# fegennari/3DWorld

Measured on AMD Instinct MI355X. Metric: heightmap Gcells/sec (noise+erosion), 16384^2 grid, higher is better.
Workload: dtype f32

## Files before the change

### 3dworld_amd/csrc/terra_common.hpp

```cpp
#pragma once
#include <stdint.h>
#include <math.h>
#include <float.h>
#include <limits.h>
#include <string.h>

#if defined(__HIPCC__)
#include <hip/hip_runtime.h>
#define TERRA_HD __host__ __device__ __forceinline__
#define TERRA_D  __device__ __forceinline__
#define TERRA_HD_COLD __host__ __device__ __attribute__((noinline))
#define TERRA_LAMBDA __host__ __device__
#else
#define TERRA_HD inline
#define TERRA_HD_COLD inline
#define TERRA_D  inline
#define TERRA_LAMBDA
#endif

#define TERRA_LIKELY(x)   __builtin_expect(!!(x), 1)
#define TERRA_UNLIKELY(x) __builtin_expect(!!(x), 0)

namespace terra {

constexpr int   F_TABLE_SIZE   = 90;
constexpr int   NUM_FREQ_COMP  = 9;
constexpr int   N_RAND_SIN2    = 10;
constexpr int   TSIZE          = 1 << 15;
constexpr float PI_F           = 3.141592654f;
constexpr int   EROSION_PAD    = 4;

TERRA_HD constexpr int sg_chunk_len(int kstart, int KC) {int const nk = F_TABLE_SIZE - kstart, n = (nk + KC - 1)/KC; return (nk > 0 && n > 0) ? (nk + n - 1)/n : 0;}
TERRA_HD constexpr int sg_chunk_last_row(int k0, int kn) {return k0 + kn - 1 + (kn & 1);}
TERRA_HD constexpr int sg_last_row_read(int kstart, int KC) {
	int const per = sg_chunk_len(kstart, KC);
	int last = -1;
	for (int k0 = kstart; per > 0 && k0 < F_TABLE_SIZE; k0 += per) {
		int const kn = (k0 + per > F_TABLE_SIZE) ? F_TABLE_SIZE - k0 : per, l = sg_chunk_last_row(k0, kn);
		if (l > last) {last = l;}
	}
	return last;
}
constexpr int SG_TABLE_ROWS = F_TABLE_SIZE + 1;
constexpr bool sg_table_rows_suffice() {
	constexpr int kcs[3] = {20, 27, 45};
	for (int i = 0; i < 3; ++i) {for (int kstart = 0; kstart <= F_TABLE_SIZE; ++kstart) {if (sg_last_row_read(kstart, kcs[i]) >= SG_TABLE_ROWS) return false;}}
	return true;
}
static_assert(sg_table_rows_suffice(), "k_sine_grid's staging would read behind the sine tables");

enum {MGEN_SINE = 0, MGEN_SIMPLEX, MGEN_PERLIN, MGEN_SIMPLEX_GPU, MGEN_DWARP_GPU};

TERRA_HD float min_std(float a, float b) {return (b < a) ? b : a;}
TERRA_HD float max_std(float a, float b) {return (a < b) ? b : a;}
TERRA_HD uint32_t f2ord(float f) {uint32_t u; memcpy(&u, &f, 4); return (u & 0x80000000u) ? ~u : (u | 0x80000000u);}
TERRA_HD float ord2f(uint32_t o) {uint32_t u = (o & 0x80000000u) ? (o & 0x7FFFFFFFu) : ~o; float f; memcpy(&f, &u, 4); return f;}
TERRA_HD int   imin(int a, int b) {return (b < a) ? b : a;}
TERRA_HD int   imax(int a, int b) {return (a < b) ? b : a;}
TERRA_HD float clip01(float x)  {return max_std(0.0f, min_std(1.0f, x));}
TERRA_HD float clip_pm1(float x) {return max_std(-1.0f, min_std(1.0f, x));}
TERRA_HD int f2i_x86(float f) {return (f >= -2147483648.0f && f < 2147483648.0f) ? (int)f : INT_MIN;}
TERRA_HD int d2i_x86(double v) {return (v > -2147483649.0 && v < 2147483648.0) ? (int)v : INT_MIN;}
TERRA_HD uint32_t f2u_x86(float f) {return (f > -9223372036854775808.0f && f < 9223372036854775808.0f) ? (uint32_t)(uint64_t)(int64_t)f : 0u;}
TERRA_HD uint32_t d2u_x86(double d) {return (d > -9223372036854775808.0 && d < 9223372036854775808.0) ? (uint32_t)(uint64_t)(int64_t)d : 0u;}
TERRA_HD int add_wrap(int a, int b) {return (int)((uint32_t)a + (uint32_t)b);}
TERRA_HD int sub_wrap(int a, int b) {return (int)((uint32_t)a - (uint32_t)b);}
TERRA_HD int abs_x86(int v) {return (v < 0) ? (int)(0u - (uint32_t)v) : v;}

struct shadow_pt_t {float x, y, z;};
TERRA_HD int shadow_region(shadow_pt_t v, float const d[3][2]) {
	int region = 0;
	if (v.x < d[0][0]) {region |= 0x01;} else if (v.x >= d[0][1]) {region |= 0x02;}
	if (v.y < d[1][0]) {region |= 0x04;} else if (v.y >= d[1][1]) {region |= 0x08;}
	if (v.z < d[2][0]) {region |= 0x10;} else if (v.z >= d[2][1]) {region |= 0x20;}
	return region;
}
TERRA_HD bool shadow_line_clip(shadow_pt_t &v1, shadow_pt_t &v2, float const d[3][2]) {
	int const region1 = shadow_region(v1, d), region2 = shadow_region(v2, d);
	if (region1 & region2) return false;
	int const region3 = region1 | region2;
	if (region3 == 0) return true;
	float tmin = 0.0f, tmax = 1.0f;
	shadow_pt_t const dv = {v2.x - v1.x, v2.y - v1.y, v2.z - v1.z};
#define TERRA_SH_CLIP(reg, va, vb, vd, vc) if (region3 & (reg)) {float const t = ((va) - (vb))/(vd); if ((vc) > 0.0f) {if (t > tmin) tmin = t;} else {if (t < tmax) tmax = t;} if (tmin >= tmax) return false;}
	TERRA_SH_CLIP(0x01, d[0][0], v1.x, dv.x,  dv.x)
	TERRA_SH_CLIP(0x02, d[0][1], v1.x, dv.x, -dv.x)
	TERRA_SH_CLIP(0x04, d[1][0], v1.y, dv.y,  dv.y)
	TERRA_SH_CLIP(0x08, d[1][1], v1.y, dv.y, -dv.y)
	TERRA_SH_CLIP(0x10, d[2][0], v1.z, dv.z,  dv.z)
	TERRA_SH_CLIP(0x20, d[2][1], v1.z, dv.z, -dv.z)
#undef TERRA_SH_CLIP
	if ((double)tmax > 1.0E-12) {v2.x = v1.x + dv.x*tmax; v2.y = v1.y + dv.y*tmax; v2.z = v1.z + dv.z*tmax;}
	if ((double)tmin < (1.0 - 1.0E-12)) {v1.x += dv.x*tmin; v1.y += dv.y*tmin; v1.z += dv.z*tmin;}
	return true;
}
template<class REMOVED, class MOVE> TERRA_HD uint32_t remove_elements_serial(uint32_t size, REMOVED removed, MOVE move) {
	for (uint32_t i = 0; i < size; ++i) {
		if (!removed(i)) continue;
		move(i, size - 1);
		--size;
		--i;
	}
	return size;
}

struct rand_gen_t {
	int64_t rseed1, rseed2;
	TERRA_HD void set_state(int64_t s1, int64_t s2) {rseed1 = s1; rseed2 = s2;}
	TERRA_HD void advance() {
		if ((rseed1 = 40014*(rseed1%53668) - 12211*(rseed1/53668)) < 0) rseed1 += 2147483563;
		if ((rseed2 = 40692*(rseed2%52774) - 3791 *(rseed2/52774)) < 0) rseed2 += 2147483399;
	}
	TERRA_HD int rand() {
		advance();
		int v = (int)rseed1 - (int)rseed2;
		if (v < 1) v += 2147483562;
		return v;
	}
	TERRA_HD double randd() {
		advance();
		double v = (double)rseed1 - (double)rseed2;
		if (v < 1) v += 2147483562;
		return v/2147483563.;
	}
	TERRA_HD float rand_float() {return (float)(0.000001*(rand()%1000000));}
	TERRA_HD float rand_uniform(float a, float b) {return a + (b - a)*(float)randd();}
};

struct sin_lut_t {
	float const *tab;
	float sscale;
	TERRA_HD int st_scale(float v) const {return f2i_x86(sscale*v) & (TSIZE-1);}
// ... 19 lines not shown
```

### 3dworld_amd/csrc/terra_hip.hip

```cpp
#include "terra_kernels.hpp"
#include "terra_fused.hpp"
#include "terra_fz_api.hpp"
#include "terra_simple_paths.hpp"
#include "terra_xfer.hpp"
#include <stdlib.h>

#define TERRA_HIP_CHECK(expr) do {hipError_t const e_ = (expr); if (e_ != hipSuccess) {throw std::runtime_error(std::string(#expr) + ": " + hipGetErrorString(e_));}} while (0)

struct hip_backend_t : terra::simple_paths<hip_backend_t> {
	int device = -1;
	hipStream_t stream = nullptr, own_stream = nullptr;
	hipEvent_t ev0 = nullptr, ev1 = nullptr;
	static constexpr bool has_kernels = true;
	terra::options_t const *opt = nullptr;
	int num_cus = 256;
	terra::dev_buf_t tile_pad, tile_order, tile_acc, tile_map, vox_p, h3_tab;
	template<class F> void for_each_buf(F f) {for (terra::dev_buf_t *b : {&tile_pad, &tile_order, &tile_acc, &tile_map, &vox_p, &h3_tab}) {f(*b);}}

	static int device_count() {int n = 0; if (hipGetDeviceCount(&n) != hipSuccess) return 0; return n;}
	void init(int dev) {
		device = dev;
		TERRA_HIP_CHECK(hipSetDevice(dev));
		TERRA_HIP_CHECK(hipStreamCreateWithFlags(&own_stream, hipStreamNonBlocking));
		stream = own_stream;
// ... 166 lines not shown
	template<class F> static void with_noise_mode(int md, F f) {
		switch (md) {
		case terra::MGEN_PERLIN:      f(std::integral_constant<int, terra::MGEN_PERLIN>()); break;
		case terra::MGEN_DWARP_GPU:   f(std::integral_constant<int, terra::MGEN_DWARP_GPU>()); break;
		case terra::MGEN_SIMPLEX_GPU: f(std::integral_constant<int, terra::MGEN_SIMPLEX_GPU>()); break;
		default:                      f(std::integral_constant<int, terra::MGEN_SIMPLEX>()); break;
		}
	}

	template<class F> void launch(size_t n, F f, int block = 256) {
		if (n == 0) return;
		use();
		size_t const nblocks = (n + block - 1)/block;
		if (nblocks > 0x7FFFFFFFull) throw std::invalid_argument("launch: grid too large");
		run(terra::k_generic<F>, dim3((unsigned)nblocks), dim3(block), 0, n, f);
	}

	template<class F> void launch_waves(size_t n, F f) {
		if (n == 0) return;
		use();
		if (n > 0x7FFFFFFFull) throw std::invalid_argument("launch_waves: grid too large");
		run(terra::k_waves<F>, dim3((unsigned)n), dim3(64), 0, f, 0u);
	}

	template<class F> void launch_waves_lean(size_t n, F f) {
		if (n == 0) return;
		use();
		if (n > 0x7FFFFFFFull) throw std::invalid_argument("launch_waves: grid too large");
		run(terra::k_waves_lean<F>, dim3((unsigned)n), dim3(64), 0, f);
	}

	template<class F> void launch_waves_nolds(size_t n, F f) {
		if (n == 0) return;
		use();
		if (n > 0x7FFFFFFFull) throw std::invalid_argument("launch_waves: grid too large");
		run(terra::k_waves_nolds<F>, dim3((unsigned)n), dim3(64), 0, f);
	}

	static float h3_scale(float amax) {int e = 0; if (amax > 0.0f && amax < 3.0e38f) {(void)frexpf(amax, &e);} return ldexpf(1.0f, 14 - e);}
	template<int KIND> bool sine_grid_h3(terra::sgf_job_t J, float amax_x, float amax_y, float const *vox_tab = nullptr, uint32_t vnx = 0, uint32_t vny = 0) {
		int const nk = (J.kstart < J.kend) ? J.kend - J.kstart : 0;
		uint32_t const nchunks = (uint32_t)((3*nk + 15)/16);
		if ((uint64_t)std::max(J.nxp, J.nyp)*32u*(nchunks + 1) >= 0xFFFFFFFFull) return false;
		size_t const bx = (size_t)nchunks*J.nxp*32u, by = (size_t)nchunks*J.nyp*32u;
		float const sx = h3_scale(amax_x), sy = h3_scale(amax_y);
		J.xh = h3_tab.grow(*this, bx + by + 64); J.yh = (char const *)J.xh + bx; J.nchunks = nchunks; J.unscale = 1.0f/(sx*sy);
		if (nchunks && vox_tab) {
			run(terra::k_split_voxel_table<false, terra::VOX_SINES>, dim3((J.nxp + 255)/256), dim3(256), 0, vox_tab, vnx, vny, J.nx, J.nxp, sx, (terra::sgh_u4 *)J.xh);
			run(terra::k_split_voxel_table<true, terra::VOX_SINES>, dim3((J.nyp + 255)/256), dim3(256), 0, vox_tab, vnx, vny, J.nx, J.nyp, sy, (terra::sgh_u4 *)J.yh);
		}
		else if (nchunks) {
			run(terra::k_split_table<false>, dim3((unsigned)(((size_t)nchunks*J.nxp + 255)/256)), dim3(256), 0, J.xt, J.nxp, J.kstart, J.kend, nchunks, sx, (terra::sgh_u4 *)J.xh);
			run(terra::k_split_table<true>, dim3((unsigned)(((size_t)nchunks*J.nyp + 255)/256)), dim3(256), 0, J.yt, J.nyp, J.kstart, J.kend, nchunks, sy, (terra::sgh_u4 *)J.yh);
		}
		if (KIND == terra::SGF_VOXELS && J.nx <= 64 && (J.nyp % 256u) == 0) {J.narrow = 1; J.ntx = 1; J.nty = J.nyp/256u;}
		unsigned const nb = J.ntx*J.nty, grid = ((nb + 7)/8)*8;
		run(terra::k_sine_grid_h3<KIND>, dim3(grid), dim3(256), 0, J);
		return true;
	}
	terra::sgf_job_t make_sgf_job(terra::grid_job_t const &job, terra::noise_consts_t const &nc, float const *xt, float const *yt, float const *smx, float const *smy, float *out, uint32_t *mm, unsigned ntx, unsigned nty) const {
		terra::sgf_job_t J; memset(&J, 0, sizeof(J));
		J.xt = xt; J.yt = yt; J.smx = smx; J.smy = smy; J.out = out; J.mm = mm; J.nx = job.nx; J.ny = job.ny; J.nxp = job.nxp; J.nyp = job.nyp; J.ntx = ntx; J.nty = nty; J.rowgroup = (unsigned)opt->sg_rowgroup;
		J.kstart = job.kstart; J.kend = terra::F_TABLE_SIZE; J.glaciate = (job.glaciate && nc.glaciate) ? 1 : 0; J.sine_mag = (job.glaciate && job.use_sine_mag) ? 1 : 0;
		J.zmax_est = nc.zmax_est; J.zmax_est2 = nc.zmax_est2; J.zmax_est2_inv = nc.zmax_est2_inv; J.sine_offset = job.sine_offset;
		return J;
	}
	bool sine_grid(terra::grid_job_t const &job, terra::noise_consts_t const &nc, terra::sin_lut_t const &L, float const *xt, float const *yt, float const *smx, float const *smy, float *out, uint32_t *mm) {
		if (opt->simple_kernels) {sine_grid_simple(job, nc, L, xt, yt, smx, smy, out); return false;}
		use();
		unsigned const ntx = job.nxp/terra::SG_BX, nty_all = (job.ny + terra::SG_BY - 1)/terra::SG_BY;
		if ((job.tyn || job.ty0) && (job.fused || job.tyn == 0 || job.ty0 >= nty_all || job.tyn > nty_all - job.ty0)) throw std::invalid_argument("sine_grid: a tile-row window must lie inside the grid (the fused kernels take whole grids only)");
		unsigned const nty = job.tyn ? job.tyn : nty_all;
		unsigned const nb = ntx*nty, grid = ((nb + 7)/8)*8;
		if (job.fused) {
			terra::sgf_job_t const J = make_sgf_job(job, nc, xt, yt, smx, smy, out, mm, ntx, nty);
			if (job.fused == 2 && sine_grid_h3<terra::SGF_GRID>(J, 1.0f, job.fast_amax)) return true;
			run(terra::k_sine_grid_mx<terra::SGF_GRID>, dim3(std::min(grid, (unsigned)(2*num_cus + 7)/8*8)), dim3(256), 0, J);
			return true;
		}
		terra::sg_tiles_t const tl{nullptr, nullptr, 0, (unsigned)opt->sg_rowgroup, 0, 0, 0, 0xFFFFFFFFu, 0, 0xFFFFFFFFu, 0};
		if (job.plain_only) {
			auto const go = [&](auto kern) {run(kern, dim3(grid), dim3(terra::SG_THREADS), 0, job, nc, L, xt, yt, smx, smy, out, ntx, nty, mm, tl);};
			if ((job.nx & 3u) == 0) {
				if (opt->sg_kc == 27) go(terra::k_sine_grid<false, false, 27>); else if (opt->sg_kc == 20) go(terra::k_sine_grid<false, false, 20>); else go(terra::k_sine_grid<false, false, 45>);
			}
			else {
				if (opt->sg_kc == 27) go(terra::k_sine_grid<false, false, 27, false>); else if (opt->sg_kc == 20) go(terra::k_sine_grid<false, false, 20, false>); else go(terra::k_sine_grid<false, false, 45, false>);
			}
		}
		else                {run(terra::k_sine_grid<false, true>, dim3(grid), dim3(terra::SG_THREADS), 0, job, nc, L, xt, yt, smx, smy, out, ntx, nty, mm, tl);}
		return true;
	}
	bool noise_grid(terra::grid_job_t const &job, terra::noise_consts_t const &nc, terra::sin_lut_t const &L, float const *smx, float const *smy, float *out, uint32_t *mm, uint32_t const *nlut) {
		if (opt->simple_kernels) {noise_grid_simple(job, nc, L, smx, smy, out); return false;}
		use();
		if (job.fused) {TERRA_HIP_CHECK((hipError_t)terra_fz_noise_grid(job.mode, &job, &nc, &L, smx, smy, out, mm, nlut, (void *)stream)); return true;}
		dim3 const grid((job.nx + 127)/128, (job.ny + terra::NG_ROWS - 1)/terra::NG_ROWS), block(256);
		terra::noise_oct_t const oc = terra::make_noise_oct(nc);
		with_noise_mode(job.mode, [&](auto m) {run(terra::k_noise_grid<decltype(m)::value>, grid, block, 0, job, nc, L, smx, smy, out, mm, nlut, oc);});
		return true;
	}
	bool tile_band_ok(uint32_t n, uint32_t nux, uint32_t nuy, uint32_t twx, bool unique_tiles, bool plain_only, int md) const {
		return !opt->simple_kernels && md == terra::MGEN_SINE && unique_tiles && plain_only && (uint64_t)n*2 >= (uint64_t)nux*nuy && ((nux*twx) & 3u) == 0 && opt->sg_kc_tiles == 27 && opt->ao_bands != 0;
	}
	void tile_grid(uint32_t n, terra::tile_ref_pod_t const *refs, uint32_t nux, uint32_t nuy, float const *xt, float const *yt, uint32_t nxpv, uint32_t nypv, float const *d_sm, float const *d_m0,
		int md, int shp, int kstart, bool use_sm, float so, terra::noise_consts_t const &nc, terra::sin_lut_t const &L, float dxv, float dyv, float *zvals, bool plain_only, uint32_t tw, bool unique_tiles, bool glaciate = true, uint32_t const *nlut = nullptr, int fused = 0, float fast_amax = 0.0f,
		terra::tile_band_t const *band = nullptr)
	{
		if (!opt->simple_kernels && md != terra::MGEN_SINE) {
			use();
			terra::grid_job_t job;
			job.mx0 = 0; job.my0 = 0; job.mdx = dxv; job.mdy = dyv; job.nx = job.ny = tw; job.nxp = nxpv; job.nyp = nypv;
			job.mode = md; job.shape = shp; job.kstart = kstart; job.glaciate = glaciate ? 1 : 0; job.use_sine_mag = use_sm ? 1 : 0; job.sine_offset = so; job.plain_only = 0;
			if (fused) {TERRA_HIP_CHECK((hipError_t)terra_fz_noise_tiles(refs, n, nux, d_sm, d_m0, &job, &nc, &L, zvals, tw, nlut, (void *)stream)); return;}
			terra::noise_oct_t const oc = terra::make_noise_oct(nc);
			size_t const threads = (size_t)n*tw*((tw + 1)/2);
			dim3 const grid((unsigned)((threads + 255)/256)), block(256);
			with_noise_mode(md, [&](auto m) {run(terra::k_noise_tiles<decltype(m)::value>, grid, block, 0, refs, n, nux, d_sm, d_m0, job, nc, L, zvals, tw, nlut, oc);});
			return;
		}
		if (opt->simple_kernels || md != terra::MGEN_SINE || !unique_tiles || (uint64_t)n*2 < (uint64_t)nux*nuy || ((uintptr_t)zvals & 7)) {tile_grid_simple(n, refs, nux, nuy, xt, yt, nxpv, nypv, d_sm, d_m0, md, shp, kstart, use_sm, so, nc, L, dxv, dyv, zvals, tw, glaciate, fused); return;}
		use();
		size_t const cnt = (size_t)nux*nuy;
		int32_t *tm = (int32_t *)tile_map.grow(*this, cnt*sizeof(int32_t));
		fill32(tm, 0xFFFFFFFFu, cnt);
		launch(n, [=] TERRA_LAMBDA (size_t i) {terra::tile_ref_pod_t const r = refs[i]; tm[(size_t)r.yi*nux + r.xi] = (int32_t)i;});
		terra::grid_job_t job;
		job.mx0 = 0; job.my0 = 0; job.mdx = dxv; job.mdy = dyv; job.nx = nux*tw; job.ny = nuy*(band ? band->twy : tw); job.nxp = nxpv; job.nyp = nypv;
		job.mode = terra::MGEN_SINE; job.shape = shp; job.kstart = kstart; job.glaciate = glaciate ? 1 : 0; job.use_sine_mag = use_sm ? 1 : 0; job.sine_offset = so;
		unsigned const ntx = job.nxp/terra::SG_BX, nty = (job.ny + terra::SG_BY - 1)/terra::SG_BY, nb = ntx*nty, grid = ((nb + 7)/8)*8;
		terra::sg_tiles_t tl{tm, d_m0, nux, (unsigned)opt->sg_rowgroup, tw, tw, tw, 0xFFFFFFFFu, 0, 0xFFFFFFFFu, 0};
		if (band) {tl.twy = band->twy; tl.ostride = band->ostride; tl.xsplit = band->xsplit; tl.xgap = band->xgap; tl.ysplit = band->ysplit; tl.ygap = band->ygap; fused = 0;}
		job.plain_only = plain_only ? 1 : 0;
		if (fused && plain_only) {
			terra::sgf_job_t J = make_sgf_job(job, nc, xt, yt, d_sm, d_sm + (size_t)nux*tw, zvals, nullptr, ntx, nty);
			J.tile_map = tm; J.nux = nux; J.tw = tw;
			if (fused == 2 && sine_grid_h3<terra::SGF_TILES>(J, 1.0f, fast_amax)) return;
			run(terra::k_sine_grid_mx<terra::SGF_TILES>, dim3(std::min(grid, (unsigned)(2*num_cus + 7)/8*8)), dim3(256), 0, J);
			return;
		}
		int const kc_tiles = opt->sg_kc_tiles;
		if (plain_only && kc_tiles == 27) {run(terra::k_sine_grid<true, false, 27>, dim3(grid), dim3(terra::SG_THREADS), 0, job, nc, L, xt, yt, d_sm, d_sm + (size_t)nux*tw, zvals, ntx, nty, (uint32_t *)nullptr, tl);}
		else if (plain_only) {run(terra::k_sine_grid<true, false>, dim3(grid), dim3(terra::SG_THREADS), 0, job, nc, L, xt, yt, d_sm, d_sm + (size_t)nux*tw, zvals, ntx, nty, (uint32_t *)nullptr, tl);}
		else            {run(terra::k_sine_grid<true, true>, dim3(grid), dim3(terra::SG_THREADS), 0, job, nc, L, xt, yt, d_sm, d_sm + (size_t)nux*tw, zvals, ntx, nty, (uint32_t *)nullptr, tl);}
	}
	terra::shadow_consts_t lanes_key; uint32_t lanes_np = 0; bool lanes_ok = false; terra::shadow_lanes_t lanes_cached;
	bool shadow_lanes(terra::shadow_consts_t const &c, uint32_t np, terra::shadow_lanes_t &lanes) {
		if (lanes_np != np || memcmp(&lanes_key, &c, sizeof(c)) != 0) {
			memset(&lanes_key, 0, sizeof(lanes_key)); memcpy(&lanes_key, &c, sizeof(c)); lanes_np = np;
			lanes_ok = terra::shadow_lane_order(c, np, terra::SH_LEVEL_THREADS, lanes_cached.path);
		}
		lanes = lanes_cached;
		return lanes_ok;
	}
	bool shadow_kernels_ok(terra::shadow_consts_t const &c, uint8_t const *sm, uint32_t np, terra::shadow_lanes_t &lanes) {
		return !opt->simple_kernels && c.xsize == 130 && !((uintptr_t)sm & 3) && shadow_lanes(c, np, lanes);
	}
	bool tile_shadows_flow(terra::shadow_consts_t const &c, uint32_t ntiles, uint32_t nslots, uint32_t const *ord, int32_t const *adj, float const *z, unsigned long long *out, uint8_t *sm, uint32_t np, uint32_t *sync_words) {
		terra::shadow_lanes_t lanes;
		if (opt->shadows_levels || !shadow_kernels_ok(c, sm, np, lanes)) return false;
		use();
		fill32(sync_words, 0u, 1);
		unsigned const grid = std::min<unsigned>(ntiles, (unsigned)(2*num_cus));
		run(terra::k_tile_shadows_flow, dim3(grid), dim3(terra::SH_LEVEL_THREADS), terra::SH_LEVEL_LDS, c, nslots, ntiles, ord, adj, z, out, sm, np, sync_words, lanes);
		return true;
	}
	void tile_shadows(terra::shadow_consts_t const &c, uint32_t cnt, uint32_t const *ord, int32_t const *adj, uint32_t n, float const *z, unsigned long long *out, uint8_t *sm, uint32_t np) {
// ... 354 lines not shown
```

### 3dworld_amd/csrc/terra_kernels.hpp

```cpp
#pragma once
#include "terra_driver.hpp"
#include "terra_noise_kernels.hpp"

namespace terra {

typedef float    st_f4 __attribute__((ext_vector_type(4)));
typedef uint32_t st_u4 __attribute__((ext_vector_type(4)));

template<class F> __global__ void k_generic(size_t n, F f) {
	size_t const i = (size_t)blockIdx.x*blockDim.x + threadIdx.x;
	if (i < n) {f(i);}
}

template<class F> __global__ __launch_bounds__(64) void k_waves(F f, unsigned first) {
	__builtin_amdgcn_s_setprio(3);
	__shared__ __attribute__((aligned(16))) float win[EW*EW];
	__shared__ uint8_t dirty[EW*EW];
	__shared__ wave_shared_t sh;
	wave_scratch_t const ws{win, dirty, &sh};
	f((size_t)blockIdx.x + first, ws);
}

template<class F> __global__ __launch_bounds__(64) void k_waves_nolds(F f) {f((size_t)blockIdx.x);}

// ... 262 lines not shown
	}
	hmap_params_t const &hp = nc.hp;
	bool const plain = !GENERAL || ((job.shape == 0) && !(hp.crack_lo < hp.crack_hi) && !(hp.volcano_width > 0.0f && hp.volcano_height > 0.0f));
	float const pp_limit = min_std(hp.plat_bot, hp.crat_h);
	float smxv[SG_TX], smyv[SG_TY];
#pragma unroll
	for (int j = 0; j < SG_TX; ++j) {unsigned const x = bx0 + (j >> 2)*64 + tx*4 + (j & 3); smxv[j] = (job.use_sine_mag && x < job.nx) ? smx[x] : 0.0f;}
#pragma unroll
	for (int i = 0; i < SG_TY; ++i) {unsigned const y = by0 + (i >> 2)*64 + ty*4 + (i & 3); smyv[i] = (job.use_sine_mag && y < job.ny) ? smy[y] : 0.0f;}
	float fmn = INFINITY, fmx = -INFINITY;
	unsigned t_ux[2] = {0, 0}, t_cx[2] = {0, 0}, t_uy[4] = {0, 0, 0, 0}, t_cy[4] = {0, 0, 0, 0};
	if (TILES) {
#pragma unroll
		for (int half = 0; half < 2; ++half) {unsigned const x = bx0 + half*64 + tx*4; t_ux[half] = x/tiles.tw; t_cx[half] = x - t_ux[half]*tiles.tw;}
#pragma unroll
		for (int g = 0; g < 4; ++g) {unsigned const y = by0 + g*64 + ty*4; t_uy[g] = y/tiles.tw; t_cy[g] = y - t_uy[g]*tiles.tw;}
	}
#pragma unroll
	for (int i = 0; i < SG_TY; ++i) {
		unsigned const y = by0 + (i >> 2)*64 + ty*4 + (i & 3);
		if (y >= job.ny) continue;
#pragma unroll
		for (int half = 0; half < 2; ++half) {
			unsigned const x = bx0 + half*64 + tx*4;
			if (x >= job.nx) continue;
			float v[4];
#pragma unroll
			for (int j = 0; j < 4; ++j) {
				float z = acc[i][half*2 + (j >> 1)][j & 1];
				if (!GENERAL || (plain && !(z > pp_limit))) {
					if (job.glaciate) {
						if (nc.glaciate) {float const relh = (z + nc.zmax_est)*nc.zmax_est2_inv; z = (GENERAL ? glaciate_exp_fn(relh, nc.custom_glaciate_exp) : relh*relh*relh)*nc.zmax_est2 - nc.zmax_est;}
						if (job.use_sine_mag) {z += smxv[half*4 + j]*smyv[i] + job.sine_offset;}
					}
				}
				else if (GENERAL && x + j < job.nx) {
					if (TILES) {
						unsigned const tw = tiles.tw, ux = (x + j)/tw, uy = y/tw;
						grid_job_t jt = job; jt.mx0 = tiles.m0[ux]; jt.my0 = tiles.m0[tiles.nux + uy];
						z = finish_cell(z, jt, nc, L, smx + ux*tw, smy + uy*tw, (x + j) - ux*tw, y - uy*tw);
					}
					else {z = finish_cell(z, job, nc, L, smx, smy, x + j, y);}
				}
				else {z = 0.0f;}
				v[j] = z;
				if (x + j < job.nx) {fmn = fminf(fmn, z); fmx = fmaxf(fmx, z);}
			}
			if (TILES) {
				unsigned const tw = tiles.tw;
				unsigned uy = t_uy[i >> 2], cy = t_cy[i >> 2] + (unsigned)(i & 3);
				if (cy >= tw) {cy -= tw; ++uy;}
				if ((tw & 1u) == 0) {
#pragma unroll
					for (int j = 0; j < 4; j += 2) {
						if (x + j >= job.nx) continue;
						unsigned ux = t_ux[half], cx = t_cx[half] + (unsigned)j;
						if (cx >= tw) {cx -= tw; ++ux;}
						int const t = tiles.tile_map[uy*tiles.nux + ux];
						if (t >= 0) {*(float2 *)(out + (size_t)t*tw*tw + cy*tw + cx) = make_float2(v[j], v[j + 1]);}
					}
					continue;
				}
#pragma unroll
				for (int j = 0; j < 4; ++j) {
					if (x + j >= job.nx) continue;
					unsigned ux = t_ux[half], cx = t_cx[half] + (unsigned)j;
					if (cx >= tw) {cx -= tw; ++ux;}
					int const t = tiles.tile_map[uy*tiles.nux + ux];
					if (t >= 0) {out[(size_t)t*tw*tw + cy*tw + cx] = v[j];}
				}
				continue;
			}
			float *o = out + (size_t)y*job.nx + x;
			if (vec_ok) {*(float4 *)o = make_float4(v[0], v[1], v[2], v[3]);}
			else {
#pragma unroll
				for (int j = 0; j < 4; ++j) {if (x + j < job.nx) o[j] = v[j];}
			}
		}
	}
	if (mm) {
		if (fmn <= fmx) {mm_lo = f2ord(fmn); mm_hi = ~f2ord(fmx);}
		wave_minmax_publish(mm_lo, mm_hi, mm);
	}
}

__global__ __launch_bounds__(256) void k_tile_land_cells(float const *__restrict__ zvals, uint32_t cells, float water_thresh, uint32_t *__restrict__ land) {
	float const *z = zvals + (size_t)blockIdx.x*cells;
	uint32_t cnt = 0;
	for (uint32_t i = threadIdx.x; i < cells; i += 256) {cnt += !(z[i] < water_thresh) ? 1u : 0u;}
#pragma unroll
	for (int off = 32; off > 0; off >>= 1) {cnt += __shfl_down(cnt, off, 64);}
	if ((threadIdx.x & 63) == 0 && cnt) {atomicAdd(&land[blockIdx.x], cnt);}
}
__global__ __launch_bounds__(256) void k_tile_order_by_land(uint32_t const *__restrict__ land, uint32_t n, uint32_t *__restrict__ order) {
	__shared__ uint32_t s_land[256];
	uint32_t const i = blockIdx.x*256 + threadIdx.x;
	uint32_t const mine = (i < n) ? land[i] : 0u;
	uint32_t pos = 0;
	for (uint32_t j0 = 0; j0 < n; j0 += 256) {
		__syncthreads();
		s_land[threadIdx.x] = (j0 + threadIdx.x < n) ? land[j0 + threadIdx.x] : 0u;
		__syncthreads();
		uint32_t const cnt = (n - j0 < 256u) ? n - j0 : 256u;
		for (uint32_t e = 0; e < cnt; ++e) {uint32_t const l = s_land[e]; pos += (l > mine || (l == mine && j0 + e < i)) ? 1u : 0u;}
	}
	if (i < n) {order[pos] = i;}
}
__global__ __launch_bounds__(64) void k_tile_erosion(float *__restrict__ zvals, erosion_consts_t ec, uint32_t iters, uint32_t const *__restrict__ order, uint32_t const *__restrict__ land) {
	extern __shared__ __attribute__((aligned(16))) float te_pad[];
	int const NX = ec.NX, NY = ec.NY, xs = ec.xsize, ys = ec.ysize;
	uint32_t const tile = order ? order[blockIdx.x] : blockIdx.x;
	float *z = zvals + (size_t)tile*xs*ys;
	if (land && land[tile] == 0) {
		for (int i = threadIdx.x; i < xs*ys; i += 64) {z[i] = max_std(ec.min_zval, z[i]);}
		return;
	}
	for (int i = threadIdx.x; i < NX*NY; i += 64) {
		int const X = i % NX, Z = i / NX;
		te_pad[i] = z[(size_t)imax(imin(Z - EROSION_PAD, ys-1), 0)*xs + imax(imin(X - EROSION_PAD, xs-1), 0)];
	}
	__syncthreads();
	{
		wave_lds_mem_t m; m.pad = te_pad; m.NX = NX; m.NY = NY;
		for (uint32_t it = 0; it < iters; ++it) {simulate_droplet((int)it, m, ec);}
	}
	__syncthreads();
	for (int i = threadIdx.x; i < xs*ys; i += 64) {
		int const x = i % xs, y = i / xs;
		z[i] = max_std(ec.min_zval, te_pad[(y + EROSION_PAD)*NX + (x + EROSION_PAD)]);
	}
}

__device__ __forceinline__ uint32_t wave_min_u32(uint32_t v) {
#pragma unroll
	for (int off = 32; off > 0; off >>= 1) {uint32_t const o = __shfl_down(v, off, 64); v = (o < v) ? o : v;}
	return v;
}
__device__ __forceinline__ int wave_min_i32(int v) {
#pragma unroll
	for (int off = 32; off > 0; off >>= 1) {int const o = __shfl_down(v, off, 64); v = (o < v) ? o : v;}
	return v;
}
constexpr unsigned TP_THREADS = 256, TP_BAND_ROWS = 34, TP_ACC = 8;
constexpr float TP_EPS = 0x1p-14f;
__global__ __launch_bounds__(256) void k_tile_post_init(uint32_t *__restrict__ acc, uint32_t n) {
	uint32_t const i = blockIdx.x*blockDim.x + threadIdx.x;
	if (i >= n*TP_ACC) return;
	uint32_t const f = i % TP_ACC;
	acc[i] = (f < 2) ? 0xFFFFFFFFu : ((f < 4) ? 0x7FFFFFFFu : ((f < 6) ? 0x80000000u : 0u));
}
__device__ __forceinline__ uint32_t tp_word_exact(float zc, float zr, float zd, float dxv, float dyv, float dxy) {
	float nv[3];
	tile_normal_v(zc, zr, zd, dxv, dyv, dxy, nv);
	uint32_t const b0 = (uint8_t)(127.0*((double)nv[0] + 1.0)), b1 = (uint8_t)(127.0*((double)nv[1] + 1.0)), b2 = (uint8_t)(127.0*((double)nv[2] + 1.0));
	return b0 | (b1 << 8) | (b2 << 16);
}
__device__ __forceinline__ bool tp_word_fast(float zc, float zr, float zd, float dxv, float dyv, float dxy, float c2, uint32_t flat_word, uint32_t &word, float &s) {
	float const n0 = dyv*(zc - zr), n1 = dxv*(zc - zd);
	s = n0*n0 + n1*n1 + c2;
	float const r = rsq_approx(s);
	float const t0 = __builtin_fmaf(127.0f, n0*r, 127.0f), t1 = __builtin_fmaf(127.0f, n1*r, 127.0f), t2 = __builtin_fmaf(127.0f, dxy*r, 127.0f);
	float const lim = 0.5f - TP_EPS;
	bool const sure = (__builtin_fabsf(__builtin_amdgcn_fractf(t0) - 0.5f) < lim) & (__builtin_fabsf(__builtin_amdgcn_fractf(t1) - 0.5f) < lim) & (__builtin_fabsf(__builtin_amdgcn_fractf(t2) - 0.5f) < lim);
	bool const flat = (n0 == 0.0f) & (n1 == 0.0f);
	uint32_t const w = (uint32_t)t0 | ((uint32_t)t1 << 8) | ((uint32_t)t2 << 16);
// ... 2669 lines not shown
```

Before: 326.3.

## Add register-tiled sine grid kernel with scalar-loaded y rows for KC=27

Adds a new k_sine_grid_rs kernel for the plain-only, 4-aligned case with sg_kc==27. Each wave holds a 16-row by 4-column accumulator tile. The y-table rows are fetched through scalar dwordx16 loads and broadcast into packed f32 multiply-adds written in inline asm. X terms are staged in LDS and software-pipelined with ds_read_b128, so each x load is reused across 16 rows and per-row vector loads of y drop out. The change adds heavy hand-written asm, a raised register count, and a new static_assert to guard against table over-read.

New measurement: 339.3 (median of 6 runs). 4.0% higher.

```diff
diff --git a/3dworld_amd/csrc/terra_common.hpp b/3dworld_amd/csrc/terra_common.hpp
--- a/3dworld_amd/csrc/terra_common.hpp
+++ b/3dworld_amd/csrc/terra_common.hpp
@@ -48,6 +48,14 @@
 	return true;
 }
 static_assert(sg_table_rows_suffice(), "k_sine_grid's staging would read behind the sine tables");
+TERRA_HD constexpr int sg_rs_last_row_read(int kstart, int KC) {
+	int const per = sg_chunk_len(kstart, KC);
+	int last = -1;
+	for (int k0 = kstart; per > 0 && k0 < F_TABLE_SIZE; k0 += per) {int const kn = (k0 + per > F_TABLE_SIZE) ? F_TABLE_SIZE - k0 : per; if (k0 + kn > last) {last = k0 + kn;}}
+	return last;
+}
+constexpr bool sg_rs_table_rows_suffice() {for (int kstart = 0; kstart <= F_TABLE_SIZE; ++kstart) {if (sg_rs_last_row_read(kstart, 27) >= SG_TABLE_ROWS) return false;} return true;}
+static_assert(sg_rs_table_rows_suffice(), "k_sine_grid_rs's row prefetch would read behind the sine tables");
 
 enum {MGEN_SINE = 0, MGEN_SIMPLEX, MGEN_PERLIN, MGEN_SIMPLEX_GPU, MGEN_DWARP_GPU};
 
diff --git a/3dworld_amd/csrc/terra_hip.hip b/3dworld_amd/csrc/terra_hip.hip
--- a/3dworld_amd/csrc/terra_hip.hip
+++ b/3dworld_amd/csrc/terra_hip.hip
@@ -272,7 +272,12 @@
 		if (job.plain_only) {
 			auto const go = [&](auto kern) {run(kern, dim3(grid), dim3(terra::SG_THREADS), 0, job, nc, L, xt, yt, smx, smy, out, ntx, nty, mm, tl);};
 			if ((job.nx & 3u) == 0) {
-				if (opt->sg_kc == 27) go(terra::k_sine_grid<false, false, 27>); else if (opt->sg_kc == 20) go(terra::k_sine_grid<false, false, 20>); else go(terra::k_sine_grid<false, false, 45>);
+				if (opt->sg_kc == 27) {
+					unsigned const first = terra::job_window_first(job), end = terra::job_window_end(job);
+					unsigned const ntx2 = (job.nxp + terra::SGR_BX - 1)/terra::SGR_BX, nty2 = (end - first + terra::SGR_BY - 1)/terra::SGR_BY, nb2 = ntx2*nty2;
+					run(terra::k_sine_grid_rs<27>, dim3(((nb2 + 7)/8)*8), dim3(terra::SG_THREADS), 0, job, nc, xt, yt, smx, smy, out, ntx2, nty2, 2u*(unsigned)opt->sg_rowgroup, mm);
+				}
+				else if (opt->sg_kc == 20) go(terra::k_sine_grid<false, false, 20>); else go(terra::k_sine_grid<false, false, 45>);
 			}
 			else {
 				if (opt->sg_kc == 27) go(terra::k_sine_grid<false, false, 27, false>); else if (opt->sg_kc == 20) go(terra::k_sine_grid<false, false, 20, false>); else go(terra::k_sine_grid<false, false, 45, false>);
diff --git a/3dworld_amd/csrc/terra_kernels.hpp b/3dworld_amd/csrc/terra_kernels.hpp
--- a/3dworld_amd/csrc/terra_kernels.hpp
+++ b/3dworld_amd/csrc/terra_kernels.hpp
@@ -368,6 +368,151 @@
 	if (mm) {
 		if (fmn <= fmx) {mm_lo = f2ord(fmn); mm_hi = ~f2ord(fmx);}
 		wave_minmax_publish(mm_lo, mm_hi, mm);
+	}
+}
+
+constexpr int SGR_BX = 256, SGR_BY = 64, SGR_ROWS = 16;
+typedef unsigned sgr_u2 __attribute__((ext_vector_type(2)));
+typedef unsigned sgr_u16 __attribute__((ext_vector_type(16)));
+typedef float sgr_v4f __attribute__((ext_vector_type(4)));
+typedef sgr_u16 const __attribute__((address_space(4))) *sgr_row16_ptr;
+__device__ __forceinline__ void sgr_mul_add_8x4(sg_v2f (&acc)[SGR_ROWS][2], int r, sg_v2f x01, sg_v2f x23, sgr_u2 y01, sgr_u2 y23, sgr_u2 y45, sgr_u2 y67) {
+	sg_v2f t0, t1;
+#define TERRA_SGR_2X4(R00, R01, R10, R11, Y) \
+	"v_pk_mul_f32 %16, %18, " Y " op_sel:[0,0] op_sel_hi:[1,0]\n\t" \
+	"v_pk_mul_f32 %17, %18, " Y " op_sel:[0,1] op_sel_hi:[1,1]\n\t" \
+	"v_pk_add_f32 " R00 ", " R00 ", %16\n\t" \
+	"v_pk_add_f32 " R10 ", " R10 ", %17\n\t" \
+	"v_pk_mul_f32 %16, %19, " Y " op_sel:[0,0] op_sel_hi:[1,0]\n\t" \
+	"v_pk_mul_f32 %17, %19, " Y " op_sel:[0,1] op_sel_hi:[1,1]\n\t" \
+	"v_pk_add_f32 " R01 ", " R01 ", %16\n\t" \
+	"v_pk_add_f32 " R11 ", " R11 ", %17\n\t"
+	asm(TERRA_SGR_2X4("%0", "%1", "%2", "%3", "%20") TERRA_SGR_2X4("%4", "%5", "%6", "%7", "%21") TERRA_SGR_2X4("%8", "%9", "%10", "%11", "%22") TERRA_SGR_2X4("%12", "%13", "%14", "%15", "%23")
+	    : "+v"(acc[r][0]), "+v"(acc[r][1]), "+v"(acc[r + 1][0]), "+v"(acc[r + 1][1]), "+v"(acc[r + 2][0]), "+v"(acc[r + 2][1]), "+v"(acc[r + 3][0]), "+v"(acc[r + 3][1]),
+	      "+v"(acc[r + 4][0]), "+v"(acc[r + 4][1]), "+v"(acc[r + 5][0]), "+v"(acc[r + 5][1]), "+v"(acc[r + 6][0]), "+v"(acc[r + 6][1]), "+v"(acc[r + 7][0]), "+v"(acc[r + 7][1]),
+	      "=&v"(t0), "=&v"(t1)
+	    : "v"(x01), "v"(x23), "s"(y01), "s"(y23), "s"(y45), "s"(y67));
+#undef TERRA_SGR_2X4
+}
+__device__ __forceinline__ void sgr_accumulate_term(sg_v2f (&acc)[SGR_ROWS][2], sgr_v4f const &x, sgr_u16 const &y) {
+	sg_v2f const x01 = {x.x, x.y}, x23 = {x.z, x.w};
+	sgr_mul_add_8x4(acc, 0, x01, x23, sgr_u2{y.s0, y.s1}, sgr_u2{y.s2, y.s3}, sgr_u2{y.s4, y.s5}, sgr_u2{y.s6, y.s7});
+	sgr_mul_add_8x4(acc, 8, x01, x23, sgr_u2{y.s8, y.s9}, sgr_u2{y.sa, y.sb}, sgr_u2{y.sc, y.sd}, sgr_u2{y.se, y.sf});
+}
+template<int SEL> __device__ __forceinline__ sg_v2f sgr_pk_mul_bcast(sg_v2f a, sgr_u2 yp) {
+	sg_v2f r;
+	if (SEL) {asm("v_pk_mul_f32 %0, %1, %2 op_sel:[0,1] op_sel_hi:[1,1]" : "=v"(r) : "v"(a), "s"(yp));}
+	else     {asm("v_pk_mul_f32 %0, %1, %2 op_sel:[0,0] op_sel_hi:[1,0]" : "=v"(r) : "v"(a), "s"(yp));}
+	return r;
+}
+template<int KC> __global__ __launch_bounds__(SG_THREADS) void k_sine_grid_rs(grid_job_t job, noise_consts_t nc, float const *__restrict__ xt, float const *__restrict__ yt,
+	float const *__restrict__ smx, float const *__restrict__ smy, float *__restrict__ out, unsigned ntx, unsigned nty, unsigned rowgroup, uint32_t *__restrict__ mm)
+{
+	__shared__ __attribute__((aligned(16))) float sX[(KC + 2)*SGR_BX];
+	unsigned bxi, byi;
+	if (!sg_tile_of_block(blockIdx.x, ntx, nty, rowgroup, bxi, byi)) return;
+	byi += job.ty0*2u;
+	uint32_t mm_lo = 0xFFFFFFFFu, mm_hi = 0xFFFFFFFFu;
+	unsigned const tid = threadIdx.x, bx0 = bxi*SGR_BX, by0 = byi*SGR_BY;
+	unsigned const w = sg_wave_uniform(tid >> 6), lane = tid & 63u;
+	sg_v2f acc[SGR_ROWS][2];
+#pragma unroll
+	for (int i = 0; i < SGR_ROWS; ++i) {acc[i][0] = sg_v2f{0.0f, 0.0f}; acc[i][1] = sg_v2f{0.0f, 0.0f};}
+	int const nk = F_TABLE_SIZE - job.kstart, nchunks = (nk + KC - 1)/KC, per_chunk = sg_chunk_len(job.kstart, KC);
+	if (job.glaciate && job.use_sine_mag) {
+		if (bx0 + w*64u < job.nxp) {sg_load_to_lds<4>(smx + bx0 + w*64u + lane, sX + (KC + 1)*SGR_BX + w*64u);}
+		if (nchunks <= 0) {__syncthreads();}
+	}
+	unsigned const xcol = bx0 + lane*4u, vx = (((xcol < job.nxp) ? xcol : job.nxp - 4u) - bx0)*4u;
+	size_t const rowb = (size_t)job.nyp*4u;
+	char const *const ybase = sg_wave_uniform_ptr(yt + by0 + w*(unsigned)SGR_ROWS);
+	unsigned const la = (unsigned)(uintptr_t)(__attribute__((address_space(3))) float *)sX + lane*16u;
+	sgr_v4f xa, xb; sgr_u16 ya, yb;
+#define TERRA_SGR_NEXT(CX, CY, NX, NY, LADDR, OFF, YP) \
+	asm volatile("s_waitcnt lgkmcnt(0)\n\ts_load_dwordx16 %1, %2, 0x0" : "+s"(CY), "=&s"(NY) : "s"(YP)); \
+	asm volatile("ds_read_b128 %1, %2 offset:" #OFF : "+v"(CX), "=&v"(NX) : "v"(LADDR))
+	for (int c = 0; c < nchunks; ++c) {
+		int const k0 = job.kstart + c*per_chunk, kn = ((k0 + per_chunk > F_TABLE_SIZE) ? F_TABLE_SIZE - k0 : per_chunk);
+		if (c > 0) {__syncthreads();}
+		char const *yp = ybase + (size_t)k0*rowb;
+		asm volatile("s_load_dwordx16 %0, %1, 0x0" : "=&s"(ya) : "s"(yp));
+		{
+			char const *gx = sg_wave_uniform_ptr(xt + (size_t)(k0 + (int)w)*job.nxp + bx0);
+			for (int r = (int)w; r < kn; r += 4) {sg_load_to_lds<16>(gx + vx, sX + r*SGR_BX); gx += (size_t)job.nxp*16u;}
+		}
+		__syncthreads();
+		asm volatile("ds_read_b128 %0, %1" : "=&v"(xa) : "v"(la));
+		unsigned a = la;
+		int k = 0;
+		for (; k + 1 < kn; k += 2) {
+			TERRA_SGR_NEXT(xa, ya, xb, yb, a, 1024, yp + rowb);   sgr_accumulate_term(acc, xa, ya); __builtin_amdgcn_sched_barrier(0);
+			TERRA_SGR_NEXT(xb, yb, xa, ya, a, 2048, yp + 2*rowb); sgr_accumulate_term(acc, xb, yb); __builtin_amdgcn_sched_barrier(0);
+			a += 2048u; yp += 2*rowb;
+		}
+		asm volatile("s_waitcnt lgkmcnt(0)" : "+s"(ya)); asm volatile("" : "+v"(xa));
+		if (k < kn) {sgr_accumulate_term(acc, xa, ya); __builtin_amdgcn_sched_barrier(0);}
+	}
+#undef TERRA_SGR_NEXT
+	typedef sg_v2f v2f;
+	bool const gl = job.glaciate && nc.glaciate, sm = job.glaciate && job.use_sine_mag;
+	float4 sx = make_float4(0.0f, 0.0f, 0.0f, 0.0f);
+	sgr_u16 sy = {0u, 0u, 0u, 0u, 0u, 0u, 0u, 0u, 0u, 0u, 0u, 0u, 0u, 0u, 0u, 0u};
+	auto const islands = [&]() {sx = *(float4 const *)(sX + (KC + 1)*SGR_BX + lane*4u); sy = *(sgr_row16_ptr)(uintptr_t)(smy + by0 + w*(unsigned)SGR_ROWS);};
+	v2f const zme = {nc.zmax_est, nc.zmax_est}, inv = {nc.zmax_est2_inv, nc.zmax_est2_inv}, z2 = {nc.zmax_est2, nc.zmax_est2}, off = {job.sine_offset, job.sine_offset};
+	float fmn = INFINITY, fmx = -INFINITY;
+	if (bx0 + SGR_BX <= job.nx && by0 + SGR_BY <= job.ny && job.nx < (1u << 24)) {
+		unsigned const voff = lane*16u;
+		char *const ob = (char *)(out + (size_t)(by0 + w*(unsigned)SGR_ROWS)*job.nx + bx0);
+		size_t const rowbytes = (size_t)job.nx*4u;
+		auto const rows = [&](auto GL, auto SM) {
+			if (decltype(SM)::value) {islands();}
+#pragma unroll
+			for (int i = 0; i < SGR_ROWS; ++i) {
+				v2f z01 = acc[i][0], z23 = acc[i][1];
+				if (decltype(GL)::value) {
+					v2f const r01 = (z01 + zme)*inv, r23 = (z23 + zme)*inv;
+					z01 = ((r01*r01)*r01)*z2 - zme; z23 = ((r23*r23)*r23)*z2 - zme;
+				}
+				if (decltype(SM)::value) {
+					v2f const s01 = {sx.x, sx.y}, s23 = {sx.z, sx.w};
+					sgr_u2 const syp = {sy[i & ~1], sy[i | 1]};
+					z01 = z01 + (((i & 1) ? sgr_pk_mul_bcast<1>(s01, syp) : sgr_pk_mul_bcast<0>(s01, syp)) + off); z23 = z23 + (((i & 1) ? sgr_pk_mul_bcast<1>(s23, syp) : sgr_pk_mul_bcast<0>(s23, syp)) + off);
+				}
+				fmn = sg_min3(sg_min3(fmn, z01.x, z01.y), z23.x, z23.y);
+				fmx = sg_max3(sg_max3(fmx, z01.x, z01.y), z23.x, z23.y);
+				*(float4 *)(ob + (size_t)i*rowbytes + voff) = make_float4(z01.x, z01.y, z23.x, z23.y);
+			}
+		};
+		typedef std::true_type yes; typedef std::false_type no;
+		if (gl) {if (sm) {rows(yes(), yes());} else {rows(yes(), no());}}
+		else    {if (sm) {rows(no(), yes());} else {rows(no(), no());}}
+	}
+	else {
+		if (sm) {islands();}
+		unsigned const x = bx0 + lane*4u;
+#pragma unroll
+		for (int i = 0; i < SGR_ROWS; ++i) {
+			unsigned const y = by0 + w*(unsigned)SGR_ROWS + (unsigned)i;
+			if (y >= job.ny || x >= job.nx) continue;
+			float const syf = __uint_as_float(sy[i]);
+			v2f const syi = {syf, syf};
+			v2f z01 = acc[i][0], z23 = acc[i][1];
+			if (gl) {
+				v2f const r01 = (z01 + zme)*inv, r23 = (z23 + zme)*inv;
+				z01 = ((r01*r01)*r01)*z2 - zme; z23 = ((r23*r23)*r23)*z2 - zme;
+			}
+			if (sm) {
+				v2f const s01 = {sx.x, sx.y}, s23 = {sx.z, sx.w};
+				z01 = z01 + (s01*syi + off); z23 = z23 + (s23*syi + off);
+			}
+			fmn = sg_min3(sg_min3(fmn, z01.x, z01.y), z23.x, z23.y);
+			fmx = sg_max3(sg_max3(fmx, z01.x, z01.y), z23.x, z23.y);
+			*(float4 *)(out + (size_t)y*job.nx + x) = make_float4(z01.x, z01.y, z23.x, z23.y);
+		}
+	}
+	if (mm) {
+		if (fmn <= fmx) {mm_lo = f2ord(fmn); mm_hi = ~f2ord(fmx);}
+		wave_minmax_publish_full(mm_lo, mm_hi, mm);
 	}
 }
 
```
